# cloneofsimo/lora

Measured on AMD Instinct MI355X. Metric: train steps/sec SD1.5 rank-4 512^2 (train_lora_dreambooth.py step), higher is better.
Workload: dtype bf16

## Files before the change

include/lora_amd.h:

```cpp
#ifndef LORA_AMD_H
#define LORA_AMD_H

#include <stddef.h>
#include <stdint.h>

#ifdef __cplusplus
extern "C" {
#endif

#define LORA_AMD_ABI_VERSION 7

#define LORA_AMD_OK 0
#define LORA_AMD_EINVAL (-1)
#define LORA_AMD_ERANK (-2)
#define LORA_AMD_ELAUNCH (-3)
#define LORA_AMD_EWORKSPACE (-4)
#define LORA_AMD_EUNSUPPORTED (-5)

#define LORA_AMD_MAX_RANK 64

#define LORA_AMD_F32 0
#define LORA_AMD_F16 1
#define LORA_AMD_BF16 2

// ... 532 lines not shown

int lora_amd_layernorm_supported(int32_t K);
int lora_amd_layernorm_fwd(const void *x, const void *gamma, const void *beta, void *y, float *stats, int64_t M,
                           int32_t K, float eps, int32_t dtype, void *stream);
int lora_amd_layernorm_bwd(const void *x, const void *gout, const void *gamma, const float *stats, void *dx,
                           int64_t M, int32_t K, int32_t dtype, void *stream);
int lora_amd_add_layernorm_fwd(const void *x, const void *res, const void *gamma, const void *beta, void *sum_out,
                               void *y, float *stats, int64_t M, int32_t K, float eps, int32_t dtype, void *stream);
int lora_amd_add_layernorm_bwd(const void *x, const void *gout, const void *gsum, const void *gamma,
                               const float *stats, void *dx, int64_t M, int32_t K, int32_t dtype, void *stream);

int lora_amd_geglu_fwd(const void *y, int64_t ldy, void *out, int64_t ldo, int64_t M, int32_t inner, int32_t dtype,
                       void *stream);
int lora_amd_geglu_bwd(const void *y, int64_t ldy, const void *gout, int64_t ldg, void *gy, int64_t ldgy, int64_t M,
                       int32_t inner, int32_t dtype, void *stream);

typedef struct lora_amd_attn_short_plan {
  int32_t run_blocks;
  int32_t slabs;
  int64_t slab_bytes;
  int64_t workspace_bytes;
} lora_amd_attn_short_plan;
int lora_amd_attn_short_bwd_supported(int64_t Sq, int32_t Sk, int32_t D, int32_t dtype, const int64_t *strides_host,
                                      int32_t n_strides);
int lora_amd_attn_short_bwd_plan(int32_t B, int32_t H, int64_t Sq, int32_t Sk, int32_t D,
                                 lora_amd_attn_short_plan *plan_host);
int lora_amd_attn_short_bwd(const void *q, const int64_t *q_strides_host, const void *k,
                            const int64_t *k_strides_host, const void *v, const int64_t *v_strides_host,
                            const void *dout, const int64_t *dout_strides_host, void *dq,
                            const int64_t *dq_strides_host, void *dk, const int64_t *dk_strides_host, void *dv,
                            const int64_t *dv_strides_host, int32_t B, int32_t H, int64_t Sq, int32_t Sk, int32_t D,
                            float scale, int32_t dtype, void *workspace, size_t workspace_bytes, void *stream);

#ifdef __cplusplus
}
#endif
#endif
```

lora_amd/_C.py:

```python
from __future__ import annotations

import ctypes as C
import os
from typing import Dict, Optional, Sequence, Tuple

import torch

_HERE = os.path.dirname(os.path.abspath(__file__))
LIB_PATH = os.path.join(_HERE, "csrc", "liblora_amd.so")

OK = 0
F32, F16, BF16 = 0, 1, 2
FACTOR_RK, FACTOR_KR = 0, 1
ROUND_REFERENCE, ROUND_ONCE, ROUND_DITHER = 0, 1, 2
MAX_RANK = 64
ABI_VERSION = 7
FM_PLAN_WIDE = 2
FM_TABLE_MASKED, FM_TABLE_WIDE = 1, 2

_DT = {torch.float32: F32, torch.float16: F16, torch.bfloat16: BF16}

class HipExtensionMissing(RuntimeError):
    pass


class AttnShortPlan(C.Structure):
    c_struct = "lora_amd_attn_short_plan"
    __slots__ = ()
    _fields_ = [("run_blocks", C.c_int32), ("slabs", C.c_int32), ("slab_bytes", C.c_int64),
                ("workspace_bytes", C.c_int64)]


class FactorsSelfPlan(C.Structure):
    c_struct = "lora_amd_factors_self_plan_t"
    __slots__ = ()
    _fields_ = [("supported", C.c_int32), ("rank_tile", C.c_int32), ("nparts", C.c_int32), ("reserved", C.c_int32),
                ("up_part_floats", C.c_int64), ("down_part_floats", C.c_int64)]


class SelfSite(C.Structure):
    c_struct = "lora_amd_self_site"
    __slots__ = ()
    _fields_ = [
        ("g", C.c_void_p), ("x", C.c_void_p), ("down", C.c_void_p), ("up", C.c_void_p),
        ("up_part", C.c_void_p), ("down_part", C.c_void_p),
        ("ldg", C.c_int64), ("ldx", C.c_int64), ("M", C.c_int64),
        ("N", C.c_int32), ("K", C.c_int32), ("r", C.c_int32), ("scale", C.c_float),
        ("g_head_dim", C.c_int32), ("g_head_pad", C.c_int32), ("x_head_dim", C.c_int32), ("x_head_pad", C.c_int32),
        ("rows_per_block", C.c_int32), ("nsplit", C.c_int32), ("kt_g", C.c_int32), ("logL_g", C.c_int32),
        ("kt_x", C.c_int32), ("logL_x", C.c_int32), ("tile_g", C.c_int32), ("nct_g", C.c_int32),
        ("tile_x", C.c_int32), ("nct_x", C.c_int32),
        ("reserved0", C.c_int32), ("reserved", C.c_int32),
        ("block_begin", C.c_int64),
    ]


class FactorsMfmaPlan(C.Structure):
    c_struct = "lora_amd_factors_mfma_plan_t"
    __slots__ = ()
    _fields_ = [("supported", C.c_int32), ("lds_class", C.c_int32), ("rank_tile", C.c_int32),
                ("rows_per_block", C.c_int32), ("nparts", C.c_int32), ("lds_bytes", C.c_int32),
                ("blocks_per_wg", C.c_int32), ("reserved", C.c_int32),
# ... 164 lines not shown
    __slots__ = ()
    _fields_ = [("down", C.c_void_p), ("up", C.c_void_p), ("pf", C.c_void_p), ("pd", C.c_void_p), ("pu", C.c_void_p),
                ("r", C.c_int32), ("C_in", C.c_int32), ("C_out", C.c_int32), ("KS", C.c_int32), ("begin", C.c_int64)]


WS_MAX_SITES = 4


class WsSite(C.Structure):
    c_struct = "lora_amd_ws_site"
    __slots__ = ()
    _fields_ = [("wp", C.c_void_p), ("bias", C.c_void_p), ("y", C.c_void_p), ("down", C.c_void_p), ("up", C.c_void_p),
                ("t_out", C.c_void_p), ("ldy", C.c_int64), ("N", C.c_int32), ("r", C.c_int32),
                ("panel_begin", C.c_int32), ("flayout", C.c_int32), ("scale", C.c_float), ("t_scale", C.c_float),
                ("dropout_p", C.c_float), ("y_heads", C.c_int32), ("seed", C.c_uint64), ("offset", C.c_uint64),
                ("offset_dev", C.c_void_p)]


class ReduceDesc(C.Structure):
    c_struct = "lora_amd_reduce_desc"
    __slots__ = ()
    _fields_ = [("part", C.c_void_p), ("out", C.c_void_p), ("begin", C.c_int64), ("nparts", C.c_int32),
                ("RT", C.c_int32), ("C", C.c_int32), ("r", C.c_int32), ("layout", C.c_int32),
                ("reserved", C.c_int32), ("scale", C.c_float), ("beta", C.c_float)]


class TembSite(C.Structure):
    c_struct = "lora_amd_temb_site"
    __slots__ = ()
    _fields_ = [("weight", C.c_void_p), ("bias", C.c_void_p), ("conv_bias", C.c_void_p), ("N", C.c_int32),
                ("row_begin", C.c_int32), ("out_offset", C.c_int64)]


MIRRORS = (AttnShortPlan, FactorsSelfPlan, SelfSite, FactorsMfmaPlan, PackSite, FmSite, RaggedDesc, SubDesc,
           PlanesDesc, SplitTDesc, ResidDesc, ThinSite, ThinQSite, ThinFinishDesc, SplitDesc, MergeSite, MstepSite,
           MergeSummary, AdamWGroup, LinearPlan, ConvPlan, Conv3NhwcPlan, Conv3PackSite, WsSite, ReduceDesc, TembSite)


vp, i32, i64, f32, u64, sz = C.c_void_p, C.c_int32, C.c_int64, C.c_float, C.c_uint64, C.c_size_t
cint, cstr, P = C.c_int, C.c_char_p, C.POINTER
FUNCTIONS = (
    ("lora_amd_abi_version", cint, ()),
    ("lora_amd_last_error", cstr, ()),
    ("lora_amd_target_arch", cstr, ()),
    ("lora_amd_merge_plan", cint, (P(MergeSite), i32, i32, P(MergeSummary))),
    ("lora_amd_merge_batched", cint, (vp, i32, P(MergeSummary), i32, i32, f32, i32, vp)),
    ("lora_amd_merge_step_plan", cint, (P(MstepSite), i32, i32, P(i64))),
    ("lora_amd_merge_step", cint, (vp, i32, i64, i32, i32, f32, i32, vp)),
    ("lora_amd_merge_step_set_tuning", cint, (i32, i32)),
    ("lora_amd_rank16_mfma", cint, (i32,)),
    ("lora_amd_rank16_mfma_takes", cint, (i32, vp, i64, i64, i32, i32, i32, i32, i32)),
    ("lora_amd_merge_set_tuning", cint, (i64, i64)),
    ("lora_amd_rowdot", cint, (vp, i64, vp, vp, i64, i32, i32, i32, i32, i32, f32, vp, i32, vp)),
    ("lora_amd_rank_update", cint, (vp, i64, vp, vp, i64, i32, i32, i32, i32, i32, f32, f32, u64, u64, vp, vp)),
    ("lora_amd_rank_update_rowscale", cint, (vp, i64, vp, vp, i64, i32, i32, i32, i32, i32, f32, vp, i32, i64, f32,
        u64, u64, vp)),
    ("lora_amd_rowdot_masked", cint, (vp, i64, vp, vp, i64, i32, i32, i32, i32, i32, f32, vp, i32, f32, u64, u64,
        vp, vp)),
    ("lora_amd_colreduce_workspace", sz, (i64, i32, i32)),
    ("lora_amd_colreduce", cint, (vp, i64, vp, vp, i64, i32, i32, i32, i32, f32, f32, f32, u64, u64, vp, vp, sz, vp)),
    ("lora_amd_rowdot_batched", cint, (vp, i64, i64, vp, i64, vp, i64, i32, i64, i32, i32, i32, i32, i32, f32, vp)),
    ("lora_amd_colreduce_batched", cint, (vp, i64, i64, vp, i64, vp, i64, i32, i64, i32, i32, i32, i32, f32, vp, sz,
        vp)),
    ("lora_amd_chol_inverse_batched", cint, (vp, vp, i32, i32, f32, vp)),
    ("lora_amd_ragged_plan", cint, (i32, vp, i32, i32, P(i64), P(i64))),
    ("lora_amd_rowdot_ragged", cint, (vp, i32, i64, i32, i32, f32, vp)),
    ("lora_amd_colreduce_ragged", cint, (vp, i32, i64, i64, i32, i32, f32, vp)),
# ... 75 lines not shown
    ("lora_amd_conv3_nhwc_fwd_fused", cint, (vp, vp, vp, vp, vp, vp, vp, i32, i32, i32, i32, i32, i32, i32, f32,
        f32, u64, u64, vp, vp)),
    ("lora_amd_sum_parts", cint, (vp, i32, i64, vp, i64, vp)),
    ("lora_amd_sumsq_workspace", sz, (i64,)),
    ("lora_amd_sumsq", cint, (vp, i64, vp, vp, sz, vp)),
    ("lora_amd_clip_adamw", cint, (vp, vp, vp, vp, i64, vp, i32, vp, f32, f32, f32, f32, f32, i64, i32, vp)),
    ("lora_amd_clip_adamw_dev", cint, (vp, vp, vp, vp, i64, vp, i32, vp, f32, f32, f32, f32, f32, vp, vp, i32, vp)),
    ("lora_amd_step_advance", cint, (vp, vp)),
    ("lora_amd_loss_scale_update", cint, (vp, vp, vp, f32, f32, i32, vp)),
    ("lora_amd_ti_rows_step", cint, (vp, vp, vp, i32, i32, i32, vp, vp, vp, f32, f32, f32, f32, f32, f32, i64, f32,
        f32, vp)),
    ("lora_amd_groupnorm_workspace", sz, (i32, i32, i32, i32)),
    ("lora_amd_groupnorm_supported", cint, (i32, i32, i32, i32)),
    ("lora_amd_groupnorm_fwd", cint, (vp, vp, vp, vp, vp, vp, sz, i32, i32, i32, i32, f32, i32, i32, vp)),
    ("lora_amd_groupnorm_bwd", cint, (vp, vp, vp, vp, vp, vp, vp, sz, i32, i32, i32, i32, i32, i32, vp)),
    ("lora_amd_groupnorm_nhwc_workspace", sz, (i32, i32, i32, i32)),
    ("lora_amd_groupnorm_nhwc_fwd", cint, (vp, vp, vp, vp, vp, vp, vp, sz, i32, i32, i32, i32, f32, i32, i32, vp)),
    ("lora_amd_groupnorm_nhwc_bwd", cint, (vp, vp, vp, vp, vp, vp, sz, i32, i32, i32, i32, i32, i32, vp)),
    ("lora_amd_groupnorm_nhwc_resident", cint, (i32,)),
    ("lora_amd_groupnorm_nhwc_route", cint, (i32, i32, i32, i32, i32, i32)),
    ("lora_amd_temb_addends_supported", cint, (i32, i32, i32)),
    ("lora_amd_temb_addends", cint, (vp, i32, i64, vp, vp, i32, i32, i32, vp)),
    ("lora_amd_layernorm_supported", cint, (i32,)),
    ("lora_amd_layernorm_fwd", cint, (vp, vp, vp, vp, vp, i64, i32, f32, i32, vp)),
    ("lora_amd_layernorm_bwd", cint, (vp, vp, vp, vp, vp, i64, i32, i32, vp)),
    ("lora_amd_add_layernorm_fwd", cint, (vp, vp, vp, vp, vp, vp, vp, i64, i32, f32, i32, vp)),
    ("lora_amd_add_layernorm_bwd", cint, (vp, vp, vp, vp, vp, vp, i64, i32, i32, vp)),
    ("lora_amd_geglu_fwd", cint, (vp, i64, vp, i64, i64, i32, i32, vp)),
    ("lora_amd_geglu_bwd", cint, (vp, i64, vp, i64, vp, i64, i64, i32, i32, vp)),
    ("lora_amd_attn_short_bwd_supported", cint, (i64, i32, i32, i32, vp, i32)),
    ("lora_amd_attn_short_bwd_plan", cint, (i32, i32, i64, i32, i32, P(AttnShortPlan))),
    ("lora_amd_attn_short_bwd", cint, (vp, vp, vp, vp, vp, vp, vp, vp, vp, vp, vp, vp, vp, vp, i32, i32, i64, i32,
        i32, f32, i32, vp, sz, vp)),
)
SYMBOLS = tuple(name for name, _, _ in FUNCTIONS)


_lib: Optional[C.CDLL] = None
_load_error: Optional[str] = None


def _declare(lib: C.CDLL) -> None:
    for name, restype, argtypes in FUNCTIONS:
        fn = getattr(lib, name)
        fn.restype, fn.argtypes = restype, list(argtypes)


def load() -> Optional[C.CDLL]:
    global _lib, _load_error
    if _lib is not None or _load_error is not None:
        return _lib
    if not os.path.exists(LIB_PATH):
        _load_error = f"{LIB_PATH} not built (run `python -c 'import __graft_entry__ as g; g.build()'`)"
        return None
    try:
        lib = C.CDLL(LIB_PATH)
        _declare(lib)
        if lib.lora_amd_abi_version() != ABI_VERSION:
            raise OSError(f"ABI version {lib.lora_amd_abi_version()} != {ABI_VERSION} (rebuild: make -C lora_amd/csrc)")
        _lib = lib
    except OSError as e:
        _load_error = f"cannot load {LIB_PATH}: {e}"
    return _lib


def available() -> bool:
# ... 1760 lines not shown
    _check(require().lora_amd_temb_addends(table.table.data_ptr(), table.n, table.rows, temb.data_ptr(), out.data_ptr(),
                                           table.B, table.K, dtype_code(table.dtype), _stream()), "lora_amd_temb_addends")
    return out


def add_layernorm_fwd(x: torch.Tensor, res: torch.Tensor, gamma: torch.Tensor, beta: torch.Tensor,
                      eps: float) -> Tuple[torch.Tensor, torch.Tensor, torch.Tensor]:
    _dev_check(x, res, gamma, beta)
    K = x.shape[-1]
    M = x.numel() // K
    s, y = torch.empty_like(x), torch.empty_like(x)
    stats = torch.empty(M, 2, dtype=torch.float32, device=x.device)
    _check(require().lora_amd_add_layernorm_fwd(x.data_ptr(), res.data_ptr(), gamma.data_ptr(), beta.data_ptr(),
                                                s.data_ptr(), y.data_ptr(), stats.data_ptr(), M, K, eps,
                                                dtype_code(x.dtype), _stream()), "lora_amd_add_layernorm_fwd")
    return s, y, stats


def add_layernorm_bwd(s: torch.Tensor, gout: torch.Tensor, gsum: Optional[torch.Tensor], gamma: torch.Tensor,
                      stats: torch.Tensor) -> torch.Tensor:
    _dev_check(s, gout, gsum, gamma, stats)
    K = s.shape[-1]
    dx = torch.empty_like(s)
    _check(require().lora_amd_add_layernorm_bwd(s.data_ptr(), gout.data_ptr(), _ptr(gsum), gamma.data_ptr(),
                                                stats.data_ptr(), dx.data_ptr(), s.numel() // K, K,
                                                dtype_code(s.dtype), _stream()), "lora_amd_add_layernorm_bwd")
    return dx


def _bhs_strides(t: torch.Tensor):
    return (C.c_int64 * 3)(t.stride(0), t.stride(1), t.stride(2))


def attn_short_bwd_supported(Sq: int, Sk: int, D: int, dtype: torch.dtype, *tensors: torch.Tensor) -> bool:
    code = _DT.get(dtype)
    if code is None:
        return False
    strides = []
    for t in tensors:
        if t.dim() != 4 or t.stride(3) != 1 or t.data_ptr() % 16 != 0:
            return False
        strides += [t.stride(0), t.stride(1), t.stride(2)]
    arr = (C.c_int64 * max(1, len(strides)))(*strides)
    return bool(require().lora_amd_attn_short_bwd_supported(Sq, Sk, D, code, arr, len(strides)))


_attn_short_plans: Dict[Tuple[int, int, int, int, int], Tuple[int, int, int, int]] = {}


def attn_short_bwd_plan(B: int, H: int, Sq: int, Sk: int, D: int) -> Tuple[int, int, int, int]:
    key = (B, H, Sq, Sk, D)
    got = _attn_short_plans.get(key)
    if got is None:
        plan = AttnShortPlan()
        _check(require().lora_amd_attn_short_bwd_plan(B, H, Sq, Sk, D, C.byref(plan)), "lora_amd_attn_short_bwd_plan")
        got = _attn_short_plans[key] = (plan.run_blocks, plan.slabs, plan.slab_bytes, plan.workspace_bytes)
    return got


def attn_short_bwd(q: torch.Tensor, k: torch.Tensor, v: torch.Tensor, dout: torch.Tensor, scale: float, *,
                   need_kv: bool = True, dq: Optional[torch.Tensor] = None, dk: Optional[torch.Tensor] = None,
                   dv: Optional[torch.Tensor] = None, workspace: Optional[torch.Tensor] = None):
    _dev_check(q, k, v, dout, dq, dk, dv, workspace)
    B, H, Sq, D = q.shape
    Sk = k.shape[2]
    if k.shape != (B, H, Sk, D) or v.shape != k.shape or dout.shape != q.shape:
        raise ValueError(f"attn_short_bwd: q {tuple(q.shape)}, k {tuple(k.shape)}, v {tuple(v.shape)}, "
                         f"dout {tuple(dout.shape)}")
    dq = torch.empty_like(q) if dq is None else dq
    if need_kv:
        dk = torch.empty_like(k) if dk is None else dk
        dv = torch.empty_like(v) if dv is None else dv
    else:
        dk = dv = None
    ops_ = [q, k, v, dout, dq] + ([dk, dv] if need_kv else [])
    if any(t.dtype != q.dtype for t in ops_) or not attn_short_bwd_supported(Sq, Sk, D, q.dtype, *ops_):
        raise ValueError(f"attn_short_bwd: unsupported problem (Sq {Sq}, Sk {Sk}, D {D}, {q.dtype}, strides "
                         f"{[tuple(t.stride()) for t in ops_]})")
    ws_bytes = attn_short_bwd_plan(B, H, Sq, Sk, D)[3]
    if need_kv:
        if workspace is None:
            workspace = torch.empty(ws_bytes, dtype=torch.uint8, device=q.device)
        have = workspace.numel() * workspace.element_size()
    else:
        have = 0
    st = [_bhs_strides(t) for t in ops_]
    _check(require().lora_amd_attn_short_bwd(
        q.data_ptr(), st[0], k.data_ptr(), st[1], v.data_ptr(), st[2], dout.data_ptr(), st[3], dq.data_ptr(), st[4],
        _ptr(dk), st[5] if need_kv else None, _ptr(dv), st[6] if need_kv else None, B, H, Sq, Sk, D, float(scale),
        dtype_code(q.dtype), _ptr(workspace) if need_kv else None, have, _stream()), "lora_amd_attn_short_bwd")
    return dq, dk, dv
```

lora_amd/ops.py:

```python
from __future__ import annotations

import os

from typing import NamedTuple, Optional

import torch
import torch.nn.functional as F

from . import _C

def next_dropout_stream(device) -> tuple:
    seed = int(torch.initial_seed()) & 0xFFFFFFFFFFFFFFFF
    pool = _POOL.get("buf")
    if pool is not None and pool.device == torch.device(device):
        i = _POOL["next"]
        if i >= pool.numel():
            pool = _POOL["buf"] = torch.empty(_POOL_SIZE, dtype=torch.int64, device=device).random_(0, 1 << 62)
            i = 0
        _POOL["next"] = i + 1
        return seed, pool[i:i + 1]
    off = torch.empty(1, dtype=torch.int64, device=device).random_(0, 1 << 62)
    return seed, off


# ... 423 lines not shown
                d_up = colreduce_any(g2, t, _C.FACTOR_KR, s, p=p, seed=seed, off=off).to(up.dtype)
        if need_down:
            if sink is not None:
                colreduce_any(x2, gt, _C.FACTOR_RK, 1.0, out=sink.down_grad, beta=1.0)
            else:
                d_down = colreduce_any(x2, gt, _C.FACTOR_RK, 1.0).to(down.dtype)
        if need_x:
            dx2 = g2 @ weight
            rank_update_any_(dx2, gt, down_c, _C.FACTOR_RK, 1.0)
            dx = dx2.view(x_shape)
    dw = g2.t() @ x2 if need_w else None
    db = g2.sum(0) if (has_bias and need_b) else None
    return dx, dw, db, d_down, d_up


def _linear_backward_unpacked(ctx, g2, drop=(0.0, 0, 0)):
    x2, weight, down, up, t = ctx.saved_tensors[:5]
    x_log = unpack_heads(x2, ctx.in_heads) if ctx.in_heads else x2
    g_log = unpack_heads(g2, ctx.out_heads) if ctx.out_heads else g2
    dx, dw, db, d_down, d_up = _linear_backward(
        (x_log, weight, down, up, t, None), ctx.needs_input_grad[:5], g_log, ctx.scale, drop, ctx.sink,
        _C.fused_ok(x_log, weight.shape[0], down.shape[0]), ctx.has_bias, x_log.shape)
    if dx is not None:
        if ctx.in_heads:
            dx = pack_heads(dx, ctx.in_heads)
        dx = dx.view(*ctx.x_shape[:-1], dx.shape[-1])
    return dx, dw, db, d_down, d_up


CONCAT_GROUPS = True
CONV3_FUSED = True
MASTER_MERGE = True
ATTN_SHORT_BWD = True
TEMB_ONE_LAUNCH = True
GN_RESIDENT = True
MERGED_WIDE = True
WIDE_FACTORS = True
WIDE_DROPOUT = True
CONV3_WIDE = True


def apply_ab_overrides(spec: str, namespace: dict) -> dict:
    allowed = ("ATTN_SHORT_BWD", "CONCAT_GROUPS", "CONV3_FUSED", "CONV3_WIDE", "GN_RESIDENT", "MASTER_MERGE", "MERGED_WIDE", "TEMB_ONE_LAUNCH", "WS_HEADS", "WS_DROPOUT", "WS_DROPOUT_WIDE",
               "WS_DROPOUT_WIDE_BWD", "WIDE_FACTORS", "WIDE_DROPOUT")
    done = {}
    for item in filter(None, (s.strip() for s in spec.split(","))):
        name, _, val = item.partition("=")
        if name not in allowed:
            raise ValueError(f"LORA_AMD_AB: unknown constant {name!r} (one of {', '.join(allowed)})")
        namespace[name] = done[name] = val.strip() not in ("0", "", "false", "False")
    return done


apply_ab_overrides(os.environ.get("LORA_AMD_AB", ""), globals())
if not GN_RESIDENT and _C.load() is not None:
    _C.groupnorm_nhwc_resident(0)

MERGE_ROUNDING = _C.ROUND_ONCE if os.environ.get("LORA_AMD_MERGE_ROUNDING", "dither") == "once" else _C.ROUND_DITHER


def master_site(w: torch.Tensor, dt: torch.dtype) -> bool:
    return MASTER_MERGE and w.dtype == torch.float32 and dt in (torch.bfloat16, torch.float16) and not w.requires_grad


def _gemm_range():
    if PATH_LOG is not None:
        return torch.profiler.record_function("lora_amd::merged_gemm")
    import contextlib

    return contextlib.nullcontext()


class MergedWeights:

    def __init__(self, state=None):
        self.entries = {}
# ... 1220 lines not shown
```

lora_amd/standin/attention.py:

```python
from __future__ import annotations

import os
from typing import Optional, Tuple

import torch
import torch.distributed as dist
import torch.nn.functional as F

try:
    from torch.nn.attention import SDPBackend, sdpa_kernel
except ImportError:
    SDPBackend = sdpa_kernel = None

from .. import _C
from .._C import _TuneCache

_CHOICE = _TuneCache("sdpa")
_AGREED = set()
_TUNE = os.environ.get("LORA_AMD_SDPA_TUNE", "1") != "0"


def _padded(d: int) -> int:
    return 64 if d <= 64 else 128 if d <= 128 else 256 if d <= 256 else d


def _library(q, k, v, scale: float, backend: Optional[str]):
    if backend is None or sdpa_kernel is None or not q.is_cuda:
        return F.scaled_dot_product_attention(q, k, v, scale=scale)
    with sdpa_kernel(getattr(SDPBackend, backend)):
        return F.scaled_dot_product_attention(q, k, v, scale=scale)


class _ShortKeyBackward(torch.autograd.Function):

    @staticmethod
    def forward(ctx, q, k, v, scale, backend):
        with torch.no_grad():
            o = _library(q, k, v, scale, backend)
        ctx.save_for_backward(q, k, v)
        ctx.scale = scale
        return o

    @staticmethod
    @torch.autograd.function.once_differentiable
    def backward(ctx, go):
        q, k, v = ctx.saved_tensors
        if go.stride(-1) != 1 or any(s % 8 for s in go.stride()[:3]) or go.data_ptr() % 16:
            go = go.contiguous()
        need_kv = ctx.needs_input_grad[1] or ctx.needs_input_grad[2]
        dq, dk, dv = _C.attn_short_bwd(q, k, v, go, ctx.scale, need_kv=need_kv)
        return (dq if ctx.needs_input_grad[0] else None, dk if ctx.needs_input_grad[1] else None,
                dv if ctx.needs_input_grad[2] else None, None, None)


ROUTES = {"native_bwd": 0, "library": 0}


def _short_bwd_eligible(q, k, v) -> bool:
    from .. import ops

    return (ops.ATTN_SHORT_BWD and q.is_cuda and _C.available() and torch.is_grad_enabled()
            and (q.requires_grad or k.requires_grad or v.requires_grad)
            and q.dim() == 4 and q.dtype == k.dtype == v.dtype and k.shape == v.shape and k.shape[-1] == q.shape[-1]
            and _C.attn_short_bwd_supported(q.shape[2], k.shape[2], q.shape[3], q.dtype, q, k, v))


def _core(q, k, v, scale: float, backend: Optional[str]):
    if _short_bwd_eligible(q, k, v):
        ROUTES["native_bwd"] += 1
        return _ShortKeyBackward.apply(q, k, v, scale, backend)
    ROUTES["library"] += 1
    return _library(q, k, v, scale, backend)


def _run(q, k, v, backend: Optional[str], pad_to: int, pad_v: bool = True):
    d = q.shape[-1]
    scale = d ** -0.5
    if pad_to > d:
        q, k = F.pad(q, (0, pad_to - d)), F.pad(k, (0, pad_to - d))
        if pad_v:
            v = F.pad(v, (0, pad_to - d))
    o = _core(q, k, v, scale, backend)
    return o[..., :d] if (pad_to > d and pad_v) else o


def _pad_candidates(d: int):
    return sorted({d, -(-d // 16) * 16, -(-d // 32) * 32, _padded(d)})


def _tune(q, k, v) -> Tuple[Optional[str], int]:
    d = q.shape[-1]
    cands = [(None, d), ("EFFICIENT_ATTENTION", d)]
    for pad in _pad_candidates(d):
        if pad > d:
            cands += [("EFFICIENT_ATTENTION", pad), ("FLASH_ATTENTION", pad), ("EFFICIENT_ATTENTION", pad, False)]
    best, best_t = (None, d), float("inf")
    for cand in cands:
        try:
            qq, kk, vv = (t.detach().clone().requires_grad_(True) for t in (q, k, v))
            go = torch.randn_like(q)
            _run(qq, kk, vv, *cand).backward(go)
            t = float("inf")
            for _ in range(3):
# ... 61 lines not shown
```

Measured before the change: 38.12.

## Add fused attention backward kernel for self-attention with up to 256 keys

Adds a HIP kernel that computes the attention backward for self-attention with 81 to 256 keys. Each workgroup keeps all key scores in registers, recomputes the softmax and produces dq directly. dK and dV partials go to per-query-block fp32 slabs, which a second fold kernel reduces. It routes to this path only when Sq equals Sk, so it targets the low-resolution UNet self-attention layers (16x16 latents) that previously used the library SDPA backward. The trade-off is a large workspace and a fold pass in place of the library's flash-style backward.

```diff
diff --git a/include/lora_amd.h b/include/lora_amd.h
--- a/include/lora_amd.h
+++ b/include/lora_amd.h
@@ -588,6 +588,23 @@
                             const int64_t *dv_strides_host, int32_t B, int32_t H, int64_t Sq, int32_t Sk, int32_t D,
                             float scale, int32_t dtype, void *workspace, size_t workspace_bytes, void *stream);
 
+typedef struct lora_amd_attn_keys_plan {
+  int32_t key_chunks;
+  int32_t slabs;
+  int64_t slab_bytes;
+  int64_t workspace_bytes;
+} lora_amd_attn_keys_plan;
+int lora_amd_attn_keys_bwd_supported(int64_t Sq, int32_t Sk, int32_t D, int32_t dtype, const int64_t *strides_host,
+                                     int32_t n_strides);
+int lora_amd_attn_keys_bwd_plan(int32_t B, int32_t H, int64_t Sq, int32_t Sk, int32_t D,
+                                lora_amd_attn_keys_plan *plan_host);
+int lora_amd_attn_keys_bwd(const void *q, const int64_t *q_strides_host, const void *k,
+                           const int64_t *k_strides_host, const void *v, const int64_t *v_strides_host,
+                           const void *dout, const int64_t *dout_strides_host, void *dq,
+                           const int64_t *dq_strides_host, void *dk, const int64_t *dk_strides_host, void *dv,
+                           const int64_t *dv_strides_host, int32_t B, int32_t H, int64_t Sq, int32_t Sk, int32_t D,
+                           float scale, int32_t dtype, void *workspace, size_t workspace_bytes, void *stream);
+
 #ifdef __cplusplus
 }
 #endif
diff --git a/lora_amd/_C.py b/lora_amd/_C.py
--- a/lora_amd/_C.py
+++ b/lora_amd/_C.py
@@ -28,6 +28,13 @@
     c_struct = "lora_amd_attn_short_plan"
     __slots__ = ()
     _fields_ = [("run_blocks", C.c_int32), ("slabs", C.c_int32), ("slab_bytes", C.c_int64),
+                ("workspace_bytes", C.c_int64)]
+
+
+class AttnKeysPlan(C.Structure):
+    c_struct = "lora_amd_attn_keys_plan"
+    __slots__ = ()
+    _fields_ = [("key_chunks", C.c_int32), ("slabs", C.c_int32), ("slab_bytes", C.c_int64),
                 ("workspace_bytes", C.c_int64)]
 
 
@@ -258,7 +265,7 @@
                 ("row_begin", C.c_int32), ("out_offset", C.c_int64)]
 
 
-MIRRORS = (AttnShortPlan, FactorsSelfPlan, SelfSite, FactorsMfmaPlan, PackSite, FmSite, RaggedDesc, SubDesc,
+MIRRORS = (AttnShortPlan, AttnKeysPlan, FactorsSelfPlan, SelfSite, FactorsMfmaPlan, PackSite, FmSite, RaggedDesc, SubDesc,
            PlanesDesc, SplitTDesc, ResidDesc, ThinSite, ThinQSite, ThinFinishDesc, SplitDesc, MergeSite, MstepSite,
            MergeSummary, AdamWGroup, LinearPlan, ConvPlan, Conv3NhwcPlan, Conv3PackSite, WsSite, ReduceDesc, TembSite)
 
@@ -400,6 +407,10 @@
     ("lora_amd_attn_short_bwd_plan", cint, (i32, i32, i64, i32, i32, P(AttnShortPlan))),
     ("lora_amd_attn_short_bwd", cint, (vp, vp, vp, vp, vp, vp, vp, vp, vp, vp, vp, vp, vp, vp, i32, i32, i64, i32,
         i32, f32, i32, vp, sz, vp)),
+    ("lora_amd_attn_keys_bwd_supported", cint, (i64, i32, i32, i32, vp, i32)),
+    ("lora_amd_attn_keys_bwd_plan", cint, (i32, i32, i64, i32, i32, P(AttnKeysPlan))),
+    ("lora_amd_attn_keys_bwd", cint, (vp, vp, vp, vp, vp, vp, vp, vp, vp, vp, vp, vp, vp, vp, i32, i32, i64, i32,
+        i32, f32, i32, vp, sz, vp)),
 )
 SYMBOLS = tuple(name for name, _, _ in FUNCTIONS)
 
@@ -2226,7 +2237,7 @@
     return (C.c_int64 * 3)(t.stride(0), t.stride(1), t.stride(2))
 
 
-def attn_short_bwd_supported(Sq: int, Sk: int, D: int, dtype: torch.dtype, *tensors: torch.Tensor) -> bool:
+def _attn_bwd_supported(fn_name: str, Sq: int, Sk: int, D: int, dtype: torch.dtype, tensors) -> bool:
     code = _DT.get(dtype)
     if code is None:
         return False
@@ -2236,7 +2247,11 @@
             return False
         strides += [t.stride(0), t.stride(1), t.stride(2)]
     arr = (C.c_int64 * max(1, len(strides)))(*strides)
-    return bool(require().lora_amd_attn_short_bwd_supported(Sq, Sk, D, code, arr, len(strides)))
+    return bool(getattr(require(), fn_name)(Sq, Sk, D, code, arr, len(strides)))
+
+
+def attn_short_bwd_supported(Sq: int, Sk: int, D: int, dtype: torch.dtype, *tensors: torch.Tensor) -> bool:
+    return _attn_bwd_supported("lora_amd_attn_short_bwd_supported", Sq, Sk, D, dtype, tensors)
 
 
 _attn_short_plans: Dict[Tuple[int, int, int, int, int], Tuple[int, int, int, int]] = {}
@@ -2252,14 +2267,12 @@
     return got
 
 
-def attn_short_bwd(q: torch.Tensor, k: torch.Tensor, v: torch.Tensor, dout: torch.Tensor, scale: float, *,
-                   need_kv: bool = True, dq: Optional[torch.Tensor] = None, dk: Optional[torch.Tensor] = None,
-                   dv: Optional[torch.Tensor] = None, workspace: Optional[torch.Tensor] = None):
+def _attn_bwd(name: str, supported, plan, q, k, v, dout, scale, need_kv, dq, dk, dv, workspace):
     _dev_check(q, k, v, dout, dq, dk, dv, workspace)
     B, H, Sq, D = q.shape
     Sk = k.shape[2]
     if k.shape != (B, H, Sk, D) or v.shape != k.shape or dout.shape != q.shape:
-        raise ValueError(f"attn_short_bwd: q {tuple(q.shape)}, k {tuple(k.shape)}, v {tuple(v.shape)}, "
+        raise ValueError(f"{name}: q {tuple(q.shape)}, k {tuple(k.shape)}, v {tuple(v.shape)}, "
                          f"dout {tuple(dout.shape)}")
     dq = torch.empty_like(q) if dq is None else dq
     if need_kv:
@@ -2268,10 +2281,10 @@
     else:
         dk = dv = None
     ops_ = [q, k, v, dout, dq] + ([dk, dv] if need_kv else [])
-    if any(t.dtype != q.dtype for t in ops_) or not attn_short_bwd_supported(Sq, Sk, D, q.dtype, *ops_):
-        raise ValueError(f"attn_short_bwd: unsupported problem (Sq {Sq}, Sk {Sk}, D {D}, {q.dtype}, strides "
+    if any(t.dtype != q.dtype for t in ops_) or not supported(Sq, Sk, D, q.dtype, *ops_):
+        raise ValueError(f"{name}: unsupported problem (Sq {Sq}, Sk {Sk}, D {D}, {q.dtype}, strides "
                          f"{[tuple(t.stride()) for t in ops_]})")
-    ws_bytes = attn_short_bwd_plan(B, H, Sq, Sk, D)[3]
+    ws_bytes = plan(B, H, Sq, Sk, D)[3]
     if need_kv:
         if workspace is None:
             workspace = torch.empty(ws_bytes, dtype=torch.uint8, device=q.device)
@@ -2279,8 +2292,39 @@
     else:
         have = 0
     st = [_bhs_strides(t) for t in ops_]
-    _check(require().lora_amd_attn_short_bwd(
+    _check(getattr(require(), "lora_amd_" + name)(
         q.data_ptr(), st[0], k.data_ptr(), st[1], v.data_ptr(), st[2], dout.data_ptr(), st[3], dq.data_ptr(), st[4],
         _ptr(dk), st[5] if need_kv else None, _ptr(dv), st[6] if need_kv else None, B, H, Sq, Sk, D, float(scale),
-        dtype_code(q.dtype), _ptr(workspace) if need_kv else None, have, _stream()), "lora_amd_attn_short_bwd")
+        dtype_code(q.dtype), _ptr(workspace) if need_kv else None, have, _stream()), "lora_amd_" + name)
     return dq, dk, dv
+
+
+def attn_short_bwd(q: torch.Tensor, k: torch.Tensor, v: torch.Tensor, dout: torch.Tensor, scale: float, *,
+                   need_kv: bool = True, dq: Optional[torch.Tensor] = None, dk: Optional[torch.Tensor] = None,
+                   dv: Optional[torch.Tensor] = None, workspace: Optional[torch.Tensor] = None):
+    return _attn_bwd("attn_short_bwd", attn_short_bwd_supported, attn_short_bwd_plan, q, k, v, dout, scale, need_kv, dq, dk,
+                     dv, workspace)
+
+
+def attn_keys_bwd_supported(Sq: int, Sk: int, D: int, dtype: torch.dtype, *tensors: torch.Tensor) -> bool:
+    return _attn_bwd_supported("lora_amd_attn_keys_bwd_supported", Sq, Sk, D, dtype, tensors)
+
+
+_attn_keys_plans: Dict[Tuple[int, int, int, int, int], Tuple[int, int, int, int]] = {}
+
+
+def attn_keys_bwd_plan(B: int, H: int, Sq: int, Sk: int, D: int) -> Tuple[int, int, int, int]:
+    key = (B, H, Sq, Sk, D)
+    got = _attn_keys_plans.get(key)
+    if got is None:
+        plan = AttnKeysPlan()
+        _check(require().lora_amd_attn_keys_bwd_plan(B, H, Sq, Sk, D, C.byref(plan)), "lora_amd_attn_keys_bwd_plan")
+        got = _attn_keys_plans[key] = (plan.key_chunks, plan.slabs, plan.slab_bytes, plan.workspace_bytes)
+    return got
+
+
+def attn_keys_bwd(q: torch.Tensor, k: torch.Tensor, v: torch.Tensor, dout: torch.Tensor, scale: float, *,
+                  need_kv: bool = True, dq: Optional[torch.Tensor] = None, dk: Optional[torch.Tensor] = None,
+                  dv: Optional[torch.Tensor] = None, workspace: Optional[torch.Tensor] = None):
+    return _attn_bwd("attn_keys_bwd", attn_keys_bwd_supported, attn_keys_bwd_plan, q, k, v, dout, scale, need_kv, dq, dk, dv,
+                     workspace)
diff --git a/lora_amd/csrc/attn_keys.hip b/lora_amd/csrc/attn_keys.hip
--- /dev/null
+++ b/lora_amd/csrc/attn_keys.hip
@@ -0,0 +1,423 @@
+#include <math.h>
+
+#include "common.hpp"
+#include "mfma16.hpp"
+
+namespace lora_amd {
+namespace {
+
+constexpr int kMinKeys = 81;
+constexpr int kMaxKeys = 256;
+constexpr int kChunk = 64;
+constexpr int kChunkTiles = 4;
+constexpr int kMaxChunks = kMaxKeys / kChunk;
+constexpr int kBlockQ = 64;
+constexpr int kLd64 = 72;
+constexpr int kThreads = 256;
+
+template <class S>
+struct AttnKeysArgs {
+  const S *q, *k, *v, *go;
+  S *dq;
+  float *ws;
+  int64_t qs[3], ks[3], vs[3], gs[3], dqs[3];
+  int Sq, Sk, H, nblk, need_kv, split;
+  float scale;
+};
+
+template <class S>
+struct AttnKeysFoldArgs {
+  const float *ws;
+  S *dk, *dv;
+  int64_t dks[3], dvs[3];
+  int Sk, H, slabs, rows;
+};
+
+template <class E>
+__device__ __forceinline__ typename FmMfma<E>::frag lds_frag(const typename E::storage *img, int row, int ld, int col, bool dead) {
+  mu32x4 v = *reinterpret_cast<const mu32x4 *>(img + row * ld + (dead ? 0 : col));
+  if (dead) v = mu32x4{0u, 0u, 0u, 0u};
+  return fm_frag<E>(v);
+}
+
+template <class E>
+__device__ __forceinline__ typename FmMfma<E>::frag lds_frag_col(const typename E::storage *img, int row0, int ld, int col) {
+  union { typename FmMfma<E>::frag f; typename E::storage s[8]; } u;
+#pragma unroll
+  for (int e = 0; e < 8; ++e) u.s[e] = img[(row0 + e) * ld + col];
+  return u.f;
+}
+
+__device__ __forceinline__ int kt_col(int d, int key) { return ((((key >> 3) ^ (d >> 3)) & 7) << 3) | (key & 7); }
+
+template <class E, int D>
+__global__ __launch_bounds__(kThreads) void attn_keys_bwd_kernel(const AttnKeysArgs<typename E::storage> a) {
+  using S = typename E::storage;
+  using frag = typename FmMfma<E>::frag;
+  constexpr int LD = D + 8;
+  constexpr int CH = D / 8;
+  constexpr int KSD = (D + 31) / 32;
+  constexpr bool HALF_D = D % 32 == 16;
+  constexpr int KSK = kChunk / 32;
+  constexpr int NDT = D / 16;
+  constexpr int TPW = (NDT + 3) / 4;
+  constexpr int NLD = (64 * CH + kThreads - 1) / kThreads;
+
+  __shared__ __attribute__((aligned(16))) S Qs[kBlockQ * LD];
+  __shared__ __attribute__((aligned(16))) S Gs[kBlockQ * LD];
+  __shared__ __attribute__((aligned(16))) S KVs[kChunk * LD];
+  __shared__ __attribute__((aligned(16))) S Kt[D * kLd64];
+  __shared__ __attribute__((aligned(16))) S dSq[kBlockQ * kLd64];
+  __shared__ __attribute__((aligned(16))) S Pt[kChunk * kLd64];
+  __shared__ __attribute__((aligned(16))) S dSt[kChunk * kLd64];
+
+  const int tid = threadIdx.x, lane = tid & 63, w = tid >> 6, c = lane & 15, g = lane >> 4;
+  const int wg = blockIdx.x / a.split, z = blockIdx.x % a.split;
+  const bool own_q = z == 0;
+  const int bh = wg / a.nblk, blk = wg % a.nblk;
+  const int b = bh / a.H, h = bh % a.H;
+  const int Sq = a.Sq, Sk = a.Sk;
+  const int nc = (Sk + kChunk - 1) / kChunk;
+  const S *qb = a.q + b * a.qs[0] + h * a.qs[1];
+  const S *gb = a.go + b * a.gs[0] + h * a.gs[1];
+  const S *kb = a.k + b * a.ks[0] + h * a.ks[1];
+  const S *vb = a.v + b * a.vs[0] + h * a.vs[1];
+  S *dqb = a.dq + b * a.dqs[0] + h * a.dqs[1];
+
+  auto fetch = [&](mu32x4 (&r)[NLD], const S *base, int64_t stride, int row0, int rows) {
+#pragma unroll
+    for (int j = 0; j < NLD; ++j) {
+      const int i = tid + j * kThreads, row = i / CH, ch = i % CH;
+      const int64_t rc = min(row0 + row, rows - 1);
+      r[j] = *gl(reinterpret_cast<const mu32x4 *>(base + rc * stride + ch * 8));
+    }
+  };
+  auto put = [&](const mu32x4 (&r)[NLD], S *img, int row0, int rows) {
+#pragma unroll
+    for (int j = 0; j < NLD; ++j) {
+      const int i = tid + j * kThreads, row = i / CH, ch = i % CH;
+      if (row < 64) *reinterpret_cast<mu32x4 *>(img + row * LD + ch * 8) = row0 + row < rows ? r[j] : mu32x4{0u, 0u, 0u, 0u};
+    }
+  };
+  auto put_t = [&](const mu32x4 (&r)[NLD], int row0, int rows) {
+#pragma unroll
+    for (int j = 0; j < NLD; ++j) {
+      const int i = tid + j * kThreads, row = i / CH, ch = i % CH;
+      if (row < 64) {
+        union { mu32x4 u; S s[8]; } x;
+        x.u = row0 + row < rows ? r[j] : mu32x4{0u, 0u, 0u, 0u};
+#pragma unroll
+        for (int e = 0; e < 8; ++e) Kt[(ch * 8 + e) * kLd64 + kt_col(ch * 8 + e, row)] = x.s[e];
+      }
+    }
+  };
+
+  mu32x4 ring[kMaxChunks][NLD];
+  {
+    mu32x4 rq[NLD], rg[NLD];
+    fetch(rq, qb, a.qs[2], blk * kBlockQ, Sq);
+    fetch(ring[0], kb, a.ks[2], 0, Sk);
+    fetch(rg, gb, a.gs[2], blk * kBlockQ, Sq);
+#pragma unroll
+    for (int kc = 1; kc < kMaxChunks; ++kc)
+      if (kc < nc) fetch(ring[kc], kb, a.ks[2], kc * kChunk, Sk);
+    put(rq, Qs, blk * kBlockQ, Sq);
+    put(ring[0], KVs, 0, Sk);
+    put(rg, Gs, blk * kBlockQ, Sq);
+    fetch(ring[0], vb, a.vs[2], 0, Sk);
+  }
+  __syncthreads();
+
+  const float sl2 = a.scale * 1.4426950408889634f;
+  const bool dead_d = HALF_D && g >= 2;
+  const int qrow = 16 * w + c;
+
+  mf32x4 s[kMaxChunks][kChunkTiles], dp[kMaxChunks][kChunkTiles];
+#pragma unroll
+  for (int kc = 0; kc < kMaxChunks; ++kc)
+#pragma unroll
+    for (int t = 0; t < kChunkTiles; ++t) s[kc][t] = dp[kc][t] = mf32x4{0.f, 0.f, 0.f, 0.f};
+
+  auto scores = [&](mf32x4 (&acc)[kChunkTiles], const S *B) {
+#pragma unroll
+    for (int ks = 0; ks < KSD; ++ks) {
+      const bool dead = ks == KSD - 1 && dead_d;
+      const int col = 32 * ks + 8 * g;
+      const frag bf = lds_frag<E>(B, qrow, LD, col, dead);
+#pragma unroll
+      for (int t = 0; t < kChunkTiles; ++t) acc[t] = FmMfma<E>::mma(lds_frag<E>(KVs, 16 * t + c, LD, col, dead), bf, acc[t]);
+    }
+  };
+
+#pragma unroll
+  for (int kc = 0; kc < kMaxChunks; ++kc) {
+    if (kc < nc) {
+      scores(s[kc], Qs);
+      __syncthreads();
+      if (kc + 1 < nc) {
+        put(ring[(kc + 1) % kMaxChunks], KVs, (kc + 1) * kChunk, Sk);
+        fetch(ring[(kc + 1) % kMaxChunks], vb, a.vs[2], (kc + 1) * kChunk, Sk);
+      } else {
+        put(ring[0], KVs, 0, Sk);
+        if (own_q) fetch(ring[0], kb, a.ks[2], 0, Sk);
+      }
+      __syncthreads();
+    }
+  }
+#pragma unroll
+  for (int kc = 0; kc < kMaxChunks; ++kc) {
+    if (kc < nc) {
+      scores(dp[kc], Gs);
+      if (kc + 1 < nc) {
+        __syncthreads();
+        put(ring[(kc + 1) % kMaxChunks], KVs, (kc + 1) * kChunk, Sk);
+        if (own_q) fetch(ring[(kc + 1) % kMaxChunks], kb, a.ks[2], (kc + 1) * kChunk, Sk);
+        __syncthreads();
+      } else if (own_q) {
+        put_t(ring[0], 0, Sk);
+      }
+    }
+  }
+
+  float m = -INFINITY;
+#pragma unroll
+  for (int kc = 0; kc < kMaxChunks; ++kc)
+#pragma unroll
+    for (int t = 0; t < kChunkTiles; ++t)
+#pragma unroll
+      for (int r = 0; r < 4; ++r) {
+        const float x = (64 * kc + 16 * t + 4 * g + r < Sk) ? s[kc][t][r] * sl2 : -INFINITY;
+        s[kc][t][r] = x;
+        m = fmaxf(m, x);
+      }
+  m = fmaxf(m, __shfl_xor(m, 16, 64));
+  m = fmaxf(m, __shfl_xor(m, 32, 64));
+  float sum = 0.f;
+#pragma unroll
+  for (int kc = 0; kc < kMaxChunks; ++kc)
+#pragma unroll
+    for (int t = 0; t < kChunkTiles; ++t)
+#pragma unroll
+      for (int r = 0; r < 4; ++r) {
+        const float p = (64 * kc + 16 * t + 4 * g + r < Sk) ? exp2f(s[kc][t][r] - m) : 0.f;
+        s[kc][t][r] = p;
+        sum += p;
+      }
+  sum += __shfl_xor(sum, 16, 64);
+  sum += __shfl_xor(sum, 32, 64);
+  const float inv = 1.f / sum;
+  float delta = 0.f;
+#pragma unroll
+  for (int kc = 0; kc < kMaxChunks; ++kc)
+#pragma unroll
+    for (int t = 0; t < kChunkTiles; ++t)
+#pragma unroll
+      for (int r = 0; r < 4; ++r) {
+        s[kc][t][r] *= inv;
+        delta += s[kc][t][r] * dp[kc][t][r];
+      }
+  delta += __shfl_xor(delta, 16, 64);
+  delta += __shfl_xor(delta, 32, 64);
+
+  mf32x4 accQ[NDT];
+#pragma unroll
+  for (int dt = 0; dt < NDT; ++dt) accQ[dt] = mf32x4{0.f, 0.f, 0.f, 0.f};
+  const int rows = nc * kChunk;
+  float *slab_k = a.ws + (int64_t)wg * (2 * rows * D), *slab_v = slab_k + rows * D;
+
+#pragma unroll
+  for (int kc = 0; kc < kMaxChunks; ++kc) {
+    if (kc < nc) {
+      const bool own_kv = a.need_kv && (a.split == 1 || (kc == 0) == own_q);
+#pragma unroll
+      for (int t = 0; t < kChunkTiles; ++t) {
+        union { mu32x2 u; S e[4]; } pk;
+#pragma unroll
+        for (int r = 0; r < 4; ++r) {
+          const float ds = s[kc][t][r] * (dp[kc][t][r] - delta);
+          pk.e[r] = E::from_f(ds);
+          if (own_kv) {
+            Pt[(16 * t + 4 * g + r) * kLd64 + qrow] = E::from_f(s[kc][t][r]);
+            dSt[(16 * t + 4 * g + r) * kLd64 + qrow] = pk.e[r];
+          }
+        }
+        if (own_q) *reinterpret_cast<mu32x2 *>(dSq + qrow * kLd64 + 16 * t + 4 * g) = pk.u;
+      }
+      __syncthreads();
+
+      if (own_q) {
+        frag dsf[KSK];
+#pragma unroll
+        for (int ks = 0; ks < KSK; ++ks) dsf[ks] = lds_frag<E>(dSq, qrow, kLd64, 32 * ks + 8 * g, false);
+#pragma unroll
+        for (int dt = 0; dt < NDT; ++dt)
+#pragma unroll
+          for (int ks = 0; ks < KSK; ++ks)
+            accQ[dt] = FmMfma<E>::mma(lds_frag<E>(Kt, 16 * dt + c, kLd64, kt_col(16 * dt + c, 32 * ks + 8 * g), false), dsf[ks],
+                                      accQ[dt]);
+      }
+
+      if (own_kv) {
+#pragma unroll
+        for (int u = 0; u < TPW; ++u) {
+          const int dt = w + 4 * u;
+          if (dt < NDT) {
+#pragma unroll
+            for (int mat = 0; mat < 2; ++mat) {
+              const S *A = mat == 0 ? dSt : Pt, *Bm = mat == 0 ? Qs : Gs;
+              mf32x4 acc[kChunkTiles];
+#pragma unroll
+              for (int t = 0; t < kChunkTiles; ++t) acc[t] = mf32x4{0.f, 0.f, 0.f, 0.f};
+#pragma unroll
+              for (int ks = 0; ks < KSK; ++ks) {
+                const frag bf = lds_frag_col<E>(Bm, 32 * ks + 8 * g, LD, 16 * dt + c);
+#pragma unroll
+                for (int t = 0; t < kChunkTiles; ++t)
+                  acc[t] = FmMfma<E>::mma(lds_frag<E>(A, 16 * t + c, kLd64, 32 * ks + 8 * g, false), bf, acc[t]);
+              }
+              float *dst = mat == 0 ? slab_k : slab_v;
+              const float f = mat == 0 ? a.scale : 1.f;
+#pragma unroll
+              for (int t = 0; t < kChunkTiles; ++t)
+#pragma unroll
+                for (int r = 0; r < 4; ++r)
+                  *gl(dst + (64 * kc + 16 * t + 4 * g + r) * D + 16 * dt + c) = acc[t][r] * f;
+            }
+          }
+        }
+      }
+      if (kc + 1 < nc) {
+        __syncthreads();
+        if (own_q) put_t(ring[(kc + 1) % kMaxChunks], (kc + 1) * kChunk, Sk);
+      }
+    }
+  }
+
+  const int qi = blk * kBlockQ + qrow;
+  if (own_q && qi < Sq) {
+#pragma unroll
+    for (int dt = 0; dt < NDT; ++dt) {
+      union { mu32x2 u; S e[4]; } pk;
+#pragma unroll
+      for (int r = 0; r < 4; ++r) pk.e[r] = E::from_f(accQ[dt][r] * a.scale);
+      *gl(reinterpret_cast<mu32x2 *>(dqb + (int64_t)qi * a.dqs[2] + 16 * dt + 4 * g)) = pk.u;
+    }
+  }
+}
+
+template <class E, int D>
+__global__ __launch_bounds__(kThreads) void attn_keys_fold_kernel(const AttnKeysFoldArgs<typename E::storage> a, int64_t total) {
+  using S = typename E::storage;
+  const int64_t i = (int64_t)blockIdx.x * kThreads + threadIdx.x;
+  if (i >= total) return;
+  constexpr int C4 = D / 4;
+  const int c4 = (int)(i % C4);
+  int64_t r = i / C4;
+  const int key = (int)(r % a.Sk);
+  r /= a.Sk;
+  const int mat = (int)(r & 1);
+  const int64_t bh = r >> 1;
+  const int64_t mat_floats = (int64_t)a.rows * D;
+  const float *p = a.ws + (bh * a.slabs * 2 + mat) * mat_floats + key * D + c4 * 4;
+  float s0 = 0.f, s1 = 0.f, s2 = 0.f, s3 = 0.f;
+  for (int sl = 0; sl < a.slabs; ++sl, p += 2 * mat_floats) {
+    const float4 x = gl_ld4(p);
+    s0 += x.x; s1 += x.y; s2 += x.z; s3 += x.w;
+  }
+  union { mu32x2 u; S e[4]; } pk;
+  pk.e[0] = E::from_f(s0); pk.e[1] = E::from_f(s1); pk.e[2] = E::from_f(s2); pk.e[3] = E::from_f(s3);
+  const int b = (int)(bh / a.H), h = (int)(bh % a.H);
+  S *dst = mat == 0 ? a.dk + b * a.dks[0] + h * a.dks[1] + key * a.dks[2] : a.dv + b * a.dvs[0] + h * a.dvs[1] + key * a.dvs[2];
+  *gl(reinterpret_cast<mu32x2 *>(dst + c4 * 4)) = pk.u;
+}
+
+bool head_dim_ok(int D) { return D == 64 || D == 80 || D == 96 || D == 128 || D == 160; }
+
+}
+}
+
+using namespace lora_amd;
+
+extern "C" int lora_amd_attn_keys_bwd_supported(int64_t Sq, int32_t Sk, int32_t D, int32_t dtype,
+                                                const int64_t *strides_host, int32_t n_strides) {
+  if (Sq < 1 || Sq > (int64_t)1 << 20 || Sk < kMinKeys || Sk > kMaxKeys || !head_dim_ok(D) || dtype != LORA_AMD_BF16) return 0;
+  for (int i = 0; i < n_strides; ++i)
+    if (strides_host == nullptr || strides_host[i] < 0 || strides_host[i] % 8 != 0) return 0;
+  return 1;
+}
+
+extern "C" int lora_amd_attn_keys_bwd_plan(int32_t B, int32_t H, int64_t Sq, int32_t Sk, int32_t D,
+                                           lora_amd_attn_keys_plan *plan_host) {
+  LORA_AMD_CHECK(plan_host != nullptr, LORA_AMD_EINVAL, "attn_keys_bwd_plan: null plan");
+  LORA_AMD_CHECK(B >= 1 && H >= 1 && (int64_t)B * H <= 1 << 20, LORA_AMD_EINVAL, "attn_keys_bwd_plan: B = %d, H = %d", B, H);
+  LORA_AMD_CHECK(lora_amd_attn_keys_bwd_supported(Sq, Sk, D, LORA_AMD_BF16, nullptr, 0), LORA_AMD_EUNSUPPORTED,
+                 "attn_keys_bwd_plan: Sq = %lld, Sk = %d, D = %d unsupported", (long long)Sq, Sk, D);
+  const int64_t nblk = (Sq + kBlockQ - 1) / kBlockQ;
+  LORA_AMD_CHECK(nblk * B * H <= (int64_t)1 << 30, LORA_AMD_EUNSUPPORTED,
+                 "attn_keys_bwd_plan: %lld query blocks x %d x %d exceed one launch", (long long)nblk, B, H);
+  plan_host->key_chunks = (Sk + kChunk - 1) / kChunk;
+  plan_host->slabs = (int32_t)nblk;
+  plan_host->slab_bytes = (int64_t)2 * plan_host->key_chunks * kChunk * D * sizeof(float);
+  plan_host->workspace_bytes = plan_host->slab_bytes * plan_host->slabs * B * H;
+  return LORA_AMD_OK;
+}
+
+extern "C" int lora_amd_attn_keys_bwd(const void *q, const int64_t *q_strides_host, const void *k,
+                                      const int64_t *k_strides_host, const void *v, const int64_t *v_strides_host,
+                                      const void *dout, const int64_t *dout_strides_host, void *dq,
+                                      const int64_t *dq_strides_host, void *dk, const int64_t *dk_strides_host, void *dv,
+                                      const int64_t *dv_strides_host, int32_t B, int32_t H, int64_t Sq, int32_t Sk, int32_t D,
+                                      float scale, int32_t dtype, void *workspace, size_t workspace_bytes, void *stream) {
+  const bool need_kv = dk != nullptr || dv != nullptr;
+  LORA_AMD_CHECK(q && k && v && dout && dq && q_strides_host && k_strides_host && v_strides_host && dout_strides_host &&
+                     dq_strides_host, LORA_AMD_EINVAL, "attn_keys_bwd: null operand");
+  LORA_AMD_CHECK(!need_kv || (dk && dv && dk_strides_host && dv_strides_host), LORA_AMD_EINVAL,
+                 "attn_keys_bwd: dk and dv come together (both or neither)");
+  int64_t st[21];
+  const int64_t *src[7] = {q_strides_host, k_strides_host, v_strides_host, dout_strides_host, dq_strides_host,
+                           need_kv ? dk_strides_host : dq_strides_host, need_kv ? dv_strides_host : dq_strides_host};
+  for (int i = 0; i < 7; ++i)
+    for (int j = 0; j < 3; ++j) st[3 * i + j] = src[i][j];
+  LORA_AMD_CHECK(lora_amd_attn_keys_bwd_supported(Sq, Sk, D, dtype, st, 21), LORA_AMD_EUNSUPPORTED,
+                 "attn_keys_bwd: Sq = %lld, Sk = %d, D = %d, dtype %d or a stride that is no multiple of 8 elements",
+                 (long long)Sq, Sk, D, dtype);
+  const void *ptrs[7] = {q, k, v, dout, dq, dk, dv};
+  for (int i = 0; i < 7; ++i)
+    LORA_AMD_CHECK(((uintptr_t)ptrs[i] & 15) == 0, LORA_AMD_EINVAL, "attn_keys_bwd: operand %d is not 16-byte aligned", i);
+  lora_amd_attn_keys_plan plan;
+  const int rc = lora_amd_attn_keys_bwd_plan(B, H, Sq, Sk, D, &plan);
+  if (rc != LORA_AMD_OK) return rc;
+  if (need_kv) {
+    LORA_AMD_CHECK(workspace != nullptr && ((uintptr_t)workspace & 15) == 0, LORA_AMD_EINVAL,
+                   "attn_keys_bwd: workspace null or not 16-byte aligned");
+    LORA_AMD_CHECK(workspace_bytes >= (size_t)plan.workspace_bytes, LORA_AMD_EWORKSPACE,
+                   "attn_keys_bwd: workspace %zu < %lld bytes", workspace_bytes, (long long)plan.workspace_bytes);
+  }
+  using S = bf16_t::storage;
+  AttnKeysArgs<S> a;
+  a.q = (const S *)q; a.k = (const S *)k; a.v = (const S *)v; a.go = (const S *)dout;
+  a.dq = (S *)dq;
+  a.ws = (float *)workspace;
+  for (int j = 0; j < 3; ++j) {
+    a.qs[j] = st[j]; a.ks[j] = st[3 + j]; a.vs[j] = st[6 + j]; a.gs[j] = st[9 + j]; a.dqs[j] = st[12 + j];
+  }
+  a.Sq = (int)Sq; a.Sk = Sk; a.H = H; a.nblk = plan.slabs; a.need_kv = need_kv ? 1 : 0;
+  a.split = need_kv ? 2 : 1;
+  a.scale = scale;
+  AttnKeysFoldArgs<S> f;
+  f.ws = (const float *)workspace; f.dk = (S *)dk; f.dv = (S *)dv;
+  for (int j = 0; j < 3; ++j) { f.dks[j] = st[15 + j]; f.dvs[j] = st[18 + j]; }
+  f.Sk = Sk; f.H = H; f.slabs = plan.slabs; f.rows = plan.key_chunks * kChunk;
+  const unsigned grid = (unsigned)((int64_t)B * H * plan.slabs * a.split);
+  const int64_t fold_total = (int64_t)B * H * 2 * Sk * (D / 4);
+  const unsigned fold_grid = (unsigned)((fold_total + kThreads - 1) / kThreads);
+  hipStream_t hs = (hipStream_t)stream;
+  by_int<64, 80, 96, 128, 160>(D, [&](auto d) {
+    constexpr int DD = decltype(d)::value;
+    hipLaunchKernelGGL((attn_keys_bwd_kernel<bf16_t, DD>), dim3(grid), dim3(kThreads), 0, hs, a);
+    if (need_kv)
+      hipLaunchKernelGGL((attn_keys_fold_kernel<bf16_t, DD>), dim3(fold_grid), dim3(kThreads), 0, hs, f, fold_total);
+    return 0;
+  });
+  return check_launch("attn_keys_bwd");
+}
diff --git a/lora_amd/ops.py b/lora_amd/ops.py
--- a/lora_amd/ops.py
+++ b/lora_amd/ops.py
@@ -479,6 +479,7 @@
 CONV3_FUSED = True
 MASTER_MERGE = True
 ATTN_SHORT_BWD = True
+ATTN_KEYS_BWD = True
 TEMB_ONE_LAUNCH = True
 GN_RESIDENT = True
 MERGED_WIDE = True
@@ -488,7 +489,7 @@
 
 
 def apply_ab_overrides(spec: str, namespace: dict) -> dict:
-    allowed = ("ATTN_SHORT_BWD", "CONCAT_GROUPS", "CONV3_FUSED", "CONV3_WIDE", "GN_RESIDENT", "MASTER_MERGE", "MERGED_WIDE", "TEMB_ONE_LAUNCH", "WS_HEADS", "WS_DROPOUT", "WS_DROPOUT_WIDE",
+    allowed = ("ATTN_KEYS_BWD", "ATTN_SHORT_BWD", "CONCAT_GROUPS", "CONV3_FUSED", "CONV3_WIDE", "GN_RESIDENT", "MASTER_MERGE", "MERGED_WIDE", "TEMB_ONE_LAUNCH", "WS_HEADS", "WS_DROPOUT", "WS_DROPOUT_WIDE",
                "WS_DROPOUT_WIDE_BWD", "WIDE_FACTORS", "WIDE_DROPOUT")
     done = {}
     for item in filter(None, (s.strip() for s in spec.split(","))):
diff --git a/lora_amd/standin/attention.py b/lora_amd/standin/attention.py
--- a/lora_amd/standin/attention.py
+++ b/lora_amd/standin/attention.py
@@ -31,14 +31,14 @@
         return F.scaled_dot_product_attention(q, k, v, scale=scale)
 
 
-class _ShortKeyBackward(torch.autograd.Function):
+class _NativeBackward(torch.autograd.Function):
 
     @staticmethod
-    def forward(ctx, q, k, v, scale, backend):
+    def forward(ctx, q, k, v, scale, backend, bwd):
         with torch.no_grad():
             o = _library(q, k, v, scale, backend)
         ctx.save_for_backward(q, k, v)
-        ctx.scale = scale
+        ctx.scale, ctx.bwd = scale, bwd
         return o
 
     @staticmethod
@@ -48,27 +48,34 @@
         if go.stride(-1) != 1 or any(s % 8 for s in go.stride()[:3]) or go.data_ptr() % 16:
             go = go.contiguous()
         need_kv = ctx.needs_input_grad[1] or ctx.needs_input_grad[2]
-        dq, dk, dv = _C.attn_short_bwd(q, k, v, go, ctx.scale, need_kv=need_kv)
+        dq, dk, dv = ctx.bwd(q, k, v, go, ctx.scale, need_kv=need_kv)
         return (dq if ctx.needs_input_grad[0] else None, dk if ctx.needs_input_grad[1] else None,
-                dv if ctx.needs_input_grad[2] else None, None, None)
+                dv if ctx.needs_input_grad[2] else None, None, None, None)
 
 
 ROUTES = {"native_bwd": 0, "library": 0}
 
 
-def _short_bwd_eligible(q, k, v) -> bool:
+def _native_bwd(q, k, v):
     from .. import ops
 
-    return (ops.ATTN_SHORT_BWD and q.is_cuda and _C.available() and torch.is_grad_enabled()
+    if not ((ops.ATTN_SHORT_BWD or ops.ATTN_KEYS_BWD) and q.is_cuda and _C.available() and torch.is_grad_enabled()
             and (q.requires_grad or k.requires_grad or v.requires_grad)
-            and q.dim() == 4 and q.dtype == k.dtype == v.dtype and k.shape == v.shape and k.shape[-1] == q.shape[-1]
-            and _C.attn_short_bwd_supported(q.shape[2], k.shape[2], q.shape[3], q.dtype, q, k, v))
+            and q.dim() == 4 and q.dtype == k.dtype == v.dtype and k.shape == v.shape and k.shape[-1] == q.shape[-1]):
+        return None
+    if ops.ATTN_SHORT_BWD and _C.attn_short_bwd_supported(q.shape[2], k.shape[2], q.shape[3], q.dtype, q, k, v):
+        return _C.attn_short_bwd
+    if (ops.ATTN_KEYS_BWD and q.shape[2] == k.shape[2]
+            and _C.attn_keys_bwd_supported(q.shape[2], k.shape[2], q.shape[3], q.dtype, q, k, v)):
+        return _C.attn_keys_bwd
+    return None
 
 
 def _core(q, k, v, scale: float, backend: Optional[str]):
-    if _short_bwd_eligible(q, k, v):
+    bwd = _native_bwd(q, k, v)
+    if bwd is not None:
         ROUTES["native_bwd"] += 1
-        return _ShortKeyBackward.apply(q, k, v, scale, backend)
+        return _NativeBackward.apply(q, k, v, scale, backend, bwd)
     ROUTES["library"] += 1
     return _library(q, k, v, scale, backend)
 
```

Result: no change. 38.35 (median of 6 runs) (+0.6%).
